# octavian-ganea/equidock_public

Measured on AMD Instinct MI355X. Metric: protein-pairs/sec (fwd+bwd) per IEGMN stack, higher is better.
Workload: dtype f32; 1 GPU; B: DB5.5-sized batch of 8 pairs x (200,200) residues, k=10, 8-layer IEGMN hdim 64, 50 heads, fp32; pairs_per_gpu=8, nodes_per_gpu=3200, edges_per_gpu=32000, layers=8, parallelism=dp1, weights=PyTorch default init (seed 0), ROT key/query x40 (SURVEY.md section 8c), svd_guard_pairs=0, launch_mode=hipGraph replay

## Files before the change

equidock_public_amd/_lib.py:

```python
import ctypes as C
import os

import torch

HERE = os.path.dirname(os.path.abspath(__file__))
LIB_PATH = os.path.join(HERE, 'libequidock_hip.so')
if os.environ.get('EQD_EXP_LIBRARY'):
    LIB_PATH = os.environ['EQD_EXP_LIBRARY']

EQD_MAX_SRC = 6
ABI_VERSION = 9
PARAMS_PER_LAYER = 19
GLOBAL_PARAMS = 5

c_float_p = C.POINTER(C.c_float)
c_int_p = C.POINTER(C.c_int32)


class EqdGraph(C.Structure):
    _fields_ = [('n_pairs', C.c_int32), ('n_lig', C.c_int32), ('n_rec', C.c_int32), ('n_nodes', C.c_int32),
                ('n_edges', C.c_int32), ('n_tiles', C.c_int32), ('n_att_items', C.c_int32), ('max_seg', C.c_int32),
                ('seg_off', C.c_void_p), ('src', C.c_void_p), ('dst', C.c_void_p), ('rowptr', C.c_void_p),
                ('csc_ptr', C.c_void_p), ('csc_eid', C.c_void_p), ('tile_node', C.c_void_p),
                ('att_items', C.c_void_p), ('res_id', C.c_void_p), ('mu_r_norm', C.c_void_p), ('he', C.c_void_p),
# ... 61 lines not shown
                ('dbc1', C.c_void_p), ('dwc2', C.c_void_p), ('dbc2', C.c_void_p)]


_lib = None
_is_sim = False
profiling = False


class EquidockHipError(RuntimeError):
    pass


def _declare(lib):
    lib.eqd_abi_version.restype = C.c_int
    lib.eqd_last_error.restype = C.c_char_p
    lib.eqd_tile_edges.restype = C.c_int
    lib.eqd_is_simulator.restype = C.c_int
    lib.eqd_model_saved_bytes.restype = C.c_size_t
    lib.eqd_model_scratch_bytes.restype = C.c_size_t
    lib.eqd_atb_partial_bytes.restype = C.c_size_t
    lib.eqd_edge_message_bwd_workspace_bytes.restype = C.c_size_t
    lib.eqd_keypoint_pool_bwd_workspace_bytes.restype = C.c_size_t
    lib.eqd_clash_workspace_bytes.restype = C.c_size_t
    lib.eqd_node_update_bwd_workspace_bytes.restype = C.c_size_t
    lib.eqd_cross_attention_bwd_ds_workspace_bytes.restype = C.c_size_t
    lib.eqd_profile_name.restype = C.c_char_p
    lib.eqd_profile_us.restype = C.c_float
    lib.eqd_tunables_reload.restype = None
    for name in ('eqd_model_layer_state', 'eqd_model_lrelu_signs', 'eqd_model_head_backward', 'eqd_profile_begin', 'eqd_profile_end', 'eqd_profile_mark', 'eqd_ctx_create', 'eqd_ctx_destroy', 'eqd_model_check', 'eqd_model_forward', 'eqd_model_backward', 'eqd_linear', 'eqd_atb',
                 'eqd_edge_message_fwd', 'eqd_edge_message_bwd', 'eqd_edge_message_bwd_kernel_only',
                 'eqd_cross_attention_fwd', 'eqd_cross_attention_fwd_bf16', 'eqd_cross_attention_bwd_bf16',
                 'eqd_cross_attention_bwd', 'eqd_cross_attention_bwd_ds',
           'eqd_keypoint_pool_fwd', 'eqd_keypoint_pool_bwd', 'eqd_kabsch_fwd', 'eqd_kabsch_bwd',
                 'eqd_rigid_apply_fwd', 'eqd_rigid_apply_bwd', 'eqd_pair_losses_fwd', 'eqd_pair_losses_bwd', 'eqd_scalar_loss', 'eqd_pocket_ot_cost',
                 'eqd_pocket_ot_fwd', 'eqd_pocket_ot_bwd', 'eqd_rigid_augment', 'eqd_protein_graph_distances',
                 'eqd_protein_graph_select', 'eqd_protein_graph_edges', 'eqd_clash_iterations', 'eqd_dropout_pack_edges', 'eqd_dropout_draw',
                 'eqd_node_update_fwd', 'eqd_node_update_bwd', 'eqd_selftest_lane_exchanges'):
        getattr(lib, name).restype = C.c_int


EXPORTS = ('eqd_model_layer_state', 'eqd_model_lrelu_signs', 'eqd_model_head_backward', 'eqd_profile_begin', 'eqd_profile_end', 'eqd_profile_mark', 'eqd_profile_name', 'eqd_profile_us', 'eqd_ctx_create', 'eqd_ctx_destroy', 'eqd_abi_version', 'eqd_last_error', 'eqd_tile_edges', 'eqd_is_simulator', 'eqd_model_saved_bytes', 'eqd_model_saved_layout',
           'eqd_model_scratch_bytes', 'eqd_model_check', 'eqd_model_forward', 'eqd_model_backward', 'eqd_linear',
           'eqd_atb_partial_bytes', 'eqd_atb', 'eqd_edge_message_fwd', 'eqd_edge_message_bwd_workspace_bytes',
           'eqd_edge_message_bwd', 'eqd_edge_message_bwd_kernel_only', 'eqd_cross_attention_fwd',
           'eqd_cross_attention_bwd', 'eqd_cross_attention_bwd_ds', 'eqd_cross_attention_bwd_ds_workspace_bytes', 'eqd_cross_attention_fwd_bf16', 'eqd_cross_attention_bwd_bf16',
           'eqd_keypoint_pool_fwd', 'eqd_keypoint_pool_bwd',
           'eqd_keypoint_pool_bwd_workspace_bytes',
           'eqd_kabsch_fwd', 'eqd_kabsch_bwd', 'eqd_rigid_apply_fwd', 'eqd_rigid_apply_bwd', 'eqd_pair_losses_fwd',
           'eqd_pair_losses_bwd', 'eqd_scalar_loss', 'eqd_pocket_ot_cost', 'eqd_pocket_ot_fwd', 'eqd_pocket_ot_bwd',
           'eqd_rigid_augment', 'eqd_protein_graph_distances', 'eqd_protein_graph_select', 'eqd_protein_graph_edges',
           'eqd_clash_workspace_bytes', 'eqd_clash_iterations', 'eqd_dropout_pack_edges', 'eqd_dropout_draw',
           'eqd_tunables_reload', 'eqd_node_update_fwd', 'eqd_node_update_bwd_workspace_bytes', 'eqd_node_update_bwd',
           'eqd_selftest_lane_exchanges', 'eqd_chain_resident_proj_launches', 'eqd_selftest_node_chain_fwd', 'eqd_model_node_state',
           'eqd_chain_resident_wide_launches')


def load_library():
    global _lib, _is_sim
    if _lib is not None:
        return _lib
    if not os.path.exists(LIB_PATH):
        raise EquidockHipError(
            f"{LIB_PATH} is missing: build it with `python -m equidock_public_amd.build` (hipcc, gfx950). "
            "There is no CPU fallback for the IEGMN hot path.")
    lib = C.CDLL(LIB_PATH)
    _declare(lib)
    if lib.eqd_abi_version() != ABI_VERSION:
        raise EquidockHipError(f"ABI version mismatch: library {lib.eqd_abi_version()} != {ABI_VERSION}")
    _lib, _is_sim = lib, bool(lib.eqd_is_simulator())
    return _lib


def load_library_for_testing(path):
    global _lib, _is_sim
    lib = C.CDLL(path)
    _declare(lib)
    _lib, _is_sim = lib, bool(lib.eqd_is_simulator())
    return _lib


def unload_for_testing():
    global _lib, _is_sim
    _lib, _is_sim = None, False


tunables_generation = 0


def reload_tunables():
    global tunables_generation
    tunables_generation += 1
    if _lib is not None:
        _lib.eqd_tunables_reload()


def is_simulator():
    return _is_sim


def check(rc):
    if rc != 0:
        raise EquidockHipError(f"libequidock_hip error {rc}: {_lib.eqd_last_error().decode()}")


def require_device(t, what='tensor'):
    if _is_sim:
        if t.is_cuda:
# ... 62 lines not shown
```

equidock_public_amd/csrc/eqd_driver.hip:

```cpp
#include "eqd_common.h"

#include <vector>

#include <string.h>

namespace {

enum {
    P_W1 = 0, P_B1, P_LNG, P_LNB, P_W2, P_B2, P_WQ, P_WK, P_WV, P_WN1, P_BN1, P_NLG, P_NLB, P_WN2, P_BN2,
    P_WC1, P_BC1, P_WC2, P_BC2
};
enum { G_EMB = 0, G_WK, G_WQ, G_WM, G_BM };

struct Dims {
    int N, E, B, K, L, d0, dh;
    int d_in(int l) const { return l == 0 ? d0 : dh; }
    int d_att(int l) const { return (d_in(l) + 15) / 16 * 16; }
    int ldw1(int l) const { return 2 * d_in(l) + 27 + 15; }
    int ldwn(int l) const { return d0 + 2 * d_in(l) + dh; }
};

Dims make_dims(const EqdModelDesc* m, const EqdGraph* g) {
    Dims D;
    D.N = g->n_nodes; D.E = g->n_edges; D.B = g->n_pairs; D.K = m->n_heads; D.L = m->n_layers;
// ... 1178 lines not shown
    nc.dHout = d_h_out; nc.Wn2 = p->Wn2; nc.Wn1 = p->Wn1; nc.y_act = y_act; nc.ln_g = p->ln_g; nc.drop_mul = p->drop_mul;
    nc.dz = W.dz; nc.lnp = W.ln_part; nc.d_aggr_msg = d_aggr_msg; nc.d_aggr_cross = aggr_cross ? d_aggr_cross : nullptr;
    nc.dh0acc = d_h0; nc.d_h = d_h;
    EqdChainJob cj[EQD_CHAIN_MAXJOBS];
    const int nj = node_bwd_chain(nc, cj);
    int nb = 0;
    RC(eqd_launch_rowchain(cj, nj, rows, st, &nb));
    EqdRedSeg segs[2] = {{W.ln_part, nb, 256, d, grads->dln_g, 0, 0, 0}, {W.ln_part + 128, nb, 256, d, grads->dln_b, 0, 0, 0}};
    RC(eqd_launch_reduce_segments(segs, 2, st));
    EqdAtbJob jobs[8];
    int na = 0;
    node_update_atb_jobs(rows, p, h, aggr_msg, aggr_cross, h0, a1n, d_h_out, W.dz, grads, jobs, &na);
    return eqd_atb(jobs, na, W.atb_part, W.atb_bytes, st);
}

extern "C" int eqd_selftest_node_chain_bwd(const EqdNodeChainBwdTest* t, int* partial_rows, void* stream) {
    if (!t || !partial_rows || !t->dH_above || !t->Wn2 || !t->Wn1 || !t->y_act || !t->ln_g || !t->dz || !t->ln_part ||
        !t->d_aggr_msg || !t->d_aggr_cross || !t->dh0acc || (t->with_dh && !t->dH)) {
        eqd_set_error("eqd_selftest_node_chain_bwd: NULL argument");
        return EQD_ERR_NULL;
    }
    if (t->rows <= 0 || t->d0 < 64 || t->d0 > 80) {
        eqd_set_error("eqd_selftest_node_chain_bwd: rows=%d d0=%d", t->rows, t->d0);
        return EQD_ERR_SHAPE;
    }
    g_bf16_mode = 0;
    const int d = 64;
    EqdLinJob dhj;
    if (t->with_dh) {
        dhj = lin_job(t->rows, d, t->dH, d, t->slope, t->ln_eps);
        for (int s = 0; s < 6; ++s) {
            if (!t->dh_X[s] || !t->dh_W[s]) {
                eqd_set_error("eqd_selftest_node_chain_bwd: NULL dh source %d", s);
                return EQD_ERR_NULL;
            }
            lin_src(dhj, s, t->dh_X[s], d, d, t->dh_W[s], 1, t->dh_wcs[s]);
        }
        dhj.nsrc = 6;
        dhj.R = t->dH_above; dhj.ldr = d; dhj.beta = 1.f - t->skip_weight_h;
    }
    NodeBwdChain nc;
    nc.N = t->rows; nc.d = d; nc.da = d; nc.d0 = t->d0; nc.d_emb = 64; nc.ldn = t->d0 + 2 * d + 64; nc.dh_width = d;
    nc.slope = t->slope; nc.eps = t->ln_eps; nc.alpha = t->skip_weight_h;
    nc.dh = t->with_dh ? &dhj : nullptr;
    nc.dHout = t->with_dh ? t->dH : t->dH_above;
    nc.Wn2 = t->Wn2; nc.Wn1 = t->Wn1; nc.y_act = t->y_act; nc.ln_g = t->ln_g; nc.drop_mul = t->drop_mul;
    nc.dz = t->dz; nc.lnp = t->ln_part; nc.d_aggr_msg = t->d_aggr_msg; nc.d_aggr_cross = t->d_aggr_cross; nc.dh0acc = t->dh0acc;
    nc.d_h = nullptr;
    EqdChainJob cj[8];
    const int nj = node_bwd_chain(nc, cj);
    return eqd_launch_rowchain(cj, nj, t->rows, (hipStream_t)stream, partial_rows);
}

extern "C" int eqd_selftest_node_chain_fwd(const EqdNodeChainFwdTest* t, void* stream) {
    if (!t || !t->h || !t->aggr_msg || !t->aggr_cross || !t->h0 || !t->Wn1 || !t->Bn1 || !t->ln_g || !t->ln_b || !t->Wn2 ||
        !t->Bn2 || !t->a1n || !t->y_act || !t->h_out) {
        eqd_set_error("eqd_selftest_node_chain_fwd: NULL argument");
        return EQD_ERR_NULL;
    }
    if (t->rows <= 0 || t->d0 < 64 || t->d0 > 80 || (t->form != 0 && t->form != 1 && t->form != 5)) {
        eqd_set_error("eqd_selftest_node_chain_fwd: rows=%d d0=%d form=%d", t->rows, t->d0, t->form);
        return EQD_ERR_SHAPE;
    }
    if (t->form == 5 ? (!t->W1 || !t->B1 || !t->WQ || !t->WK || !t->WV || !t->P || !t->Q || !t->qa || !t->ka || !t->va)
                     : (t->form == 1 && (!t->WM || !t->BM || !t->hm))) {
        eqd_set_error("eqd_selftest_node_chain_fwd: NULL argument of a carried job");
        return EQD_ERR_NULL;
    }
    g_bf16_mode = 0;
    const int d = 64;
    NodeFwdChain fc;
    fc.N = t->rows; fc.d = d; fc.da = d; fc.d0 = t->d0; fc.dh = d; fc.ldn = t->d0 + 2 * d + 64; fc.ld_a1n = d;
    fc.slope = t->slope; fc.eps = t->ln_eps; fc.skip = t->skip_weight_h;
    fc.h = t->h; fc.aggr_msg = t->aggr_msg; fc.aggr_cross = t->aggr_cross; fc.h0 = t->h0;
    fc.Wn1 = t->Wn1; fc.Bn1 = t->Bn1; fc.ln_g = t->ln_g; fc.ln_b = t->ln_b; fc.Wn2 = t->Wn2; fc.Bn2 = t->Bn2;
    fc.drop_mul = t->drop_mul;
    fc.a1n = t->a1n; fc.y_act = t->y_act; fc.h_out = t->h_out; fc.a1n_b = nullptr; fc.hb_out = nullptr;
    fc.next = nullptr; fc.head = nullptr;
    NodePre np;
    EqdLinJob jm;
    if (t->form == 5) {
        np.N = t->rows; np.d = d; np.da = d; np.ldw1 = 2 * d; np.slope = t->slope; np.eps = t->ln_eps; np.cross = true;
        np.W1 = t->W1; np.B1 = t->B1; np.WQ = t->WQ; np.WK = t->WK; np.WV = t->WV;
        np.P = t->P; np.Q = t->Q; np.qa = t->qa; np.ka = t->ka; np.va = t->va;
        np.qa_b = np.ka_b = np.va_b = nullptr;
        fc.next = &np;
    } else if (t->form == 1) {
        jm = lin_job(t->rows, 64, t->hm, 64, t->slope, t->ln_eps);
        lin_src(jm, 0, t->h_out, d, d, t->WM, d, 1);
        jm.nsrc = 1; jm.bias = t->BM; jm.act = 1;
        jm.mul = t->head_mul; jm.ld_mul = 64;
        fc.head = &jm;
    }
    EqdChainJob cj[EQD_CHAIN_MAXJOBS];
    const int nj = node_fwd_chain(fc, cj);
    return eqd_launch_rowchain(cj, nj, t->rows, (hipStream_t)stream);
}
```

equidock_public_amd/csrc/eqd_node_kernels.hip:

```cpp
#include "eqd_common.h"
#include "eqd_linear_inl.h"
#include "eqd_rowwave_inl.h"
#include "eqd_rowres_inl.h"
#include "eqd_rowres80_inl.h"
#include "eqd_chainres_inl.h"
#include "eqd_chainres_wide_inl.h"
#include "eqd_gather_inl.h"

#include <atomic>
#include <mutex>
#include <vector>

#include <stdarg.h>
#include <stdio.h>
#include <stdlib.h>
#include <string.h>

static thread_local char g_err[512] = "";

void eqd_set_error(const char* fmt, ...) {
    va_list ap;
    va_start(ap, fmt);
    vsnprintf(g_err, sizeof(g_err), fmt, ap);
    va_end(ap);
// ... 499 lines not shown
    *(f32x4*)&Lb[0][out_l][l15 * LIN_S + f0] = z;
    if (rv && jY) *(EQD_GAS f4v*)&jY[(size_t)rowi * ldy + f0] = z;
    float v8[8];
#pragma unroll
    for (int r = 0; r < 4; ++r) {
        v8[r] = o[r] * xh[r];
        v8[4 + r] = o[r];
    }
    const bool b3 = (l15 & 8) != 0, b2 = (l15 & 4) != 0, b1 = (l15 & 2) != 0;
    float w4[4], w2[2];
#pragma unroll
    for (int i = 0; i < 4; ++i) w4[i] = (b3 ? v8[i + 4] : v8[i]) + lane_xor<8>(b3 ? v8[i] : v8[i + 4]);
#pragma unroll
    for (int i = 0; i < 2; ++i) w2[i] = (b2 ? w4[i + 2] : w4[i]) + lane_xor<4>(b2 ? w4[i] : w4[i + 2]);
    float w1 = (b1 ? w2[1] : w2[0]) + lane_xor<2>(b1 ? w2[0] : w2[1]);
    w1 += lane_xor<1>(w1);
    if ((l15 & 1) == 0) {
        const int idx = l15 >> 1;
        jaux[(size_t)blockIdx.x * 256 + (idx < 4 ? 0 : 128) + f0 + (idx & 3)] = w1;
    }
}
struct LnBwd64Desc {
    const JobW& W;
    bool have_y;
    f32x4 yp;
#define LJ(f) JW_OFF(EqdLinJob, f)
    __device__ __forceinline__ int rows() const { return jw_i(W, LJ(rows)); }
    __device__ __forceinline__ int src_l() const { return jw_i(W, JW_OFF(EqdChainJob, src_local)); }
    __device__ __forceinline__ int out_l() const { return jw_i(W, JW_OFF(EqdChainJob, out_local)); }
    __device__ __forceinline__ float slope() const { return jw_f(W, LJ(slope)); }
    __device__ __forceinline__ float ln_eps() const { return jw_f(W, LJ(ln_eps)); }
    __device__ __forceinline__ f32x4 gam(int f0) const { return *(const EQD_GAS f4v*)(jw_p<const float>(W, LJ(ln_g)) + f0); }
    __device__ __forceinline__ f32x4 y_act(int row, int f0) const {
        if (have_y) return yp;
        const int ldx = jw_i(W, LJ(s) + JW_OFF(EqdLinSrc, ldx));
        return *(const EQD_GAS f4v*)(jw_p<const float>(W, LJ(s) + JW_OFF(EqdLinSrc, X)) + (size_t)row * ldx + f0);
    }
    __device__ __forceinline__ float* Y() const { return jw_p<float>(W, LJ(Y)); }
    __device__ __forceinline__ int ldy() const { return jw_i(W, LJ(ldy)); }
    __device__ __forceinline__ float* aux() const { return jw_p<float>(W, JW_OFF(EqdChainJob, aux)); }
    __device__ __forceinline__ f32x4 mul(int row, int f0) const {
        f32x4 mulv = {1.f, 1.f, 1.f, 1.f};
        if (const float* const jmul = jw_p<const float>(W, LJ(mul)))
            mulv = *(const EQD_GAS f4v*)(jmul + (size_t)row * jw_i(W, LJ(ld_mul)) + f0);
        return mulv;
    }
#undef LJ
};
__device__ __forceinline__ void chain_lnbwd64(const JobW& W, float (*Lb)[LIN_LOCALS][16 * LIN_S], float (*stat)[EQD_WAVES][16],
                                              int row0, bool have_y, f32x4 yp) {
    chain_lnbwd64_t(LnBwd64Desc{W, have_y, yp}, Lb, stat, row0);
}
#include "eqd_chainres_bwd_inl.h"

template <int RT>
__device__ __forceinline__ void chain_lnbwd(const EqdChainJob& C, float (*Lb)[LIN_LOCALS][16 * LIN_S], float (*red)[256],
                                            int row0) {
    const EqdLinJob& J = C.lin;
    const EQD_GAS float* const jlng = (const EQD_GAS float*)uni(J.ln_g);
    const EQD_GAS float* const jX = (const EQD_GAS float*)uni(J.s[0].X);
    EQD_GAS float* const jY = (EQD_GAS float*)uni(J.Y);
    EQD_GAS float* const jaux = (EQD_GAS float*)uni(C.aux);
    const EQD_GAS float* const jmul = (const EQD_GAS float*)uni(J.mul);
    const int ld_mul = uni(J.ld_mul);
    const int rows = uni(J.rows), ldx = uni(J.s[0].ldx), ldy = uni(J.ldy), src_l = uni(C.src_local[0]), out_l = uni(C.out_local);
    const float slope = uni(J.slope), ln_eps = uni(J.ln_eps);
    const int t = threadIdx.x, lane = t & 63, wave = t >> 6;
    const int d = uni(J.M);
    const int f0 = lane, f1 = lane + 64;
    const bool v0 = f0 < d, v1 = f1 < d;
    const float g0 = v0 ? jlng[f0] : 0.f, g1 = v1 ? jlng[f1] : 0.f;
    const float invd = 1.f / (float)d;
    float dg0 = 0.f, dg1 = 0.f, db0 = 0.f, db1 = 0.f;
    float y0s[RT][4], y1s[RT][4];
#pragma unroll
    for (int rt = 0; rt < RT; ++rt)
#pragma unroll
        for (int rr = 0; rr < 4; ++rr) {
            int row = row0 + 16 * rt + 4 * wave + rr;
            row = row < rows ? row : rows - 1;
            const size_t o = (size_t)row * ldx;
            y0s[rt][rr] = jX[o + (v0 ? f0 : 0)];
            y1s[rt][rr] = jX[o + (v1 ? f1 : 0)];
        }
#pragma unroll
    for (int rt = 0; rt < RT; ++rt) {
        const float* __restrict__ din = Lb[rt][src_l];
        float* __restrict__ dout = Lb[rt][out_l];
#pragma unroll
        for (int rr = 0; rr < 4; ++rr) {
            const int lr = 4 * wave + rr;
            const int row = row0 + 16 * rt + lr;
            const bool rv = row < rows;
            const float y0 = (rv && v0) ? y0s[rt][rr] : 0.f, y1 = (rv && v1) ? y1s[rt][rr] : 0.f;
            const float o0 = (rv && v0) ? din[lr * LIN_S + f0] : 0.f, o1 = (rv && v1) ? din[lr * LIN_S + f1] : 0.f;
            const float mean = wave_sum(y0 + y1) * invd;
            const float c0 = v0 ? y0 - mean : 0.f, c1 = v1 ? y1 - mean : 0.f;
            const float rstd = 1.f / sqrtf(wave_sum(c0 * c0 + c1 * c1) * invd + ln_eps);
            const float xh0 = c0 * rstd, xh1 = c1 * rstd;
            const float dx0 = o0 * g0, dx1 = o1 * g1;
            const float s1 = wave_sum(dx0 + dx1) * invd;
            const float s2 = wave_sum(dx0 * xh0 + dx1 * xh1) * invd;
            float z0 = rstd * (dx0 - s1 - xh0 * s2) * lrelu_grad(y0, slope);
            float z1 = rstd * (dx1 - s1 - xh1 * s2) * lrelu_grad(y1, slope);
            if (jmul) {
                const size_t mo = (size_t)(rv ? row : rows - 1) * ld_mul;
// ... 314 lines not shown
            return false;
        for (int s = 0; s < nsrc; ++s)
            if (!J.s[s].W || J.s[s].mask || J.s[s].K != 64 || J.s[s].w_rs != 1) return false;
        return true;
    };
    auto src = [](const EqdLinSrc& S) { return CrbSrc{S.X, S.W, S.ldx, S.w_cs}; };
    auto out = [](const EqdLinJob& J) { return CrbOut{J.Y, J.R, J.ldy, J.ldr, J.alpha, J.beta}; };
    memset(&A, 0, sizeof(A));
    A.rows = rows;
    int at = 0;
    if (dh) {
        const EqdChainJob& C = jobs[at++];
        if (!plain(C, 6) || C.out_local != 2 || !C.lin.Y || !C.lin.R) return false;
        for (int s = 0; s < 6; ++s) {
            if (!C.lin.s[s].X || C.src_local[s] >= 0) return false;
            A.dh[s] = src(C.lin.s[s]);
        }
        A.dho = out(C.lin);
    }
    {
        const EqdChainJob& C = jobs[at++];
        if (!plain(C, 1) || C.out_local != 0 || C.lin.Y || C.lin.R) return false;
        if (dh ? C.src_local[0] != 2 : (C.src_local[0] >= 0 || !C.lin.s[0].X)) return false;
        A.a = src(C.lin.s[0]);
        A.a_alpha = C.lin.alpha;
        A.a_beta = C.lin.beta;
    }
    {
        const EqdChainJob& C = jobs[at++];
        const EqdLinJob& J = C.lin;
        if (C.type != 1 || J.bf16 || J.rows != rows || J.M != 64 || C.src_local[0] != 0 || C.out_local != 1 || !J.s[0].X ||
            !J.ln_g || !J.Y || !C.aux)
            return false;
        A.y_act = J.s[0].X; A.ld_y = J.s[0].ldx;
        A.ln_g = J.ln_g;
        A.mul = J.mul; A.ld_mul = J.ld_mul;
        A.dz = J.Y; A.ld_dz = J.ldy;
        A.aux = C.aux;
        A.slope = J.slope; A.ln_eps = J.ln_eps;
    }
    for (int j = 0; j < 3; ++j) {
        const EqdChainJob& C = jobs[at++];
        if (!plain(C, 1) || C.src_local[0] != 1 || C.out_local >= 0 || !C.lin.Y) return false;
        if (C.lin.R && !(dh && j == 2 && C.lin.R == C.lin.Y && C.lin.ldr == C.lin.ldy)) return false;
        A.x[j] = src(C.lin.s[0]);
        A.xo[j] = out(C.lin);
        if (j > 0 && (A.x[j].W != A.x[j - 1].W + 64 || A.x[j].wcs != A.x[j - 1].wcs)) return false;
    }
    return true;
}
static std::atomic<long long> g_chain_resident_bwd_launches{0};
extern "C" long long eqd_chain_resident_bwd_launches(void) { return g_chain_resident_bwd_launches.load(); }

enum RowBody {
    ROW_NONE,
    ROW_RES80,
    ROW_RES, ROW_WAVE,
    ROW_CRF0, ROW_CRF1, ROW_CRF5,
    ROW_CRW,
    ROW_CRB, ROW_CRB_DH,
    ROW_CHAIN
};
struct RowPlan {
    RowBody body;
    int grid;
    int tps;
    bool bf;
    int rt, occ;
    union {
        ChainResFwdArg f;
        ChainResWideArg w;
        ChainResBwdArg b;
    } res;
    std::atomic<long long>* count[2];
};
static RowPlan row_plan(const EqdChainJob* jobs, int njobs, int rows, bool chain, bool wide_ok) {
    RowPlan P;
    memset(&P, 0, sizeof(P));
    P.bf = njobs > 0 && jobs[0].lin.bf16;
    const bool rw = rw_eligible(jobs, njobs, rows);
    if (!rw && rw80_eligible(jobs, njobs, rows)) P.body = ROW_RES80;
    else if (rw) P.body = rw_mode(rows) == 2 && rr_single_tile(jobs, njobs) ? ROW_RES : ROW_WAVE;
    if (P.body == ROW_WAVE) P.grid = rw_blocks(rows);
    else if (P.body != ROW_NONE) { P.tps = rr_tiles_per_wg(rows); P.grid = rr_blocks(rows); }
    if (P.body != ROW_NONE || !chain) return P;
    P.grid = eqd_rowchain_blocks(rows);
    const int occ = rowchain_occ_forced();
    if (cr_rows_ok(rows, occ)) {
        int np = 0;
        if (crf_pack(jobs, njobs, rows, P.res.f, np)) {
            P.body = np == 5 ? ROW_CRF5 : np == 1 ? ROW_CRF1 : ROW_CRF0;
            P.count[0] = &g_chain_resident_launches;
            if (np) P.count[1] = &g_chain_resident_proj_launches;
            return P;
        }
        if (wide_ok && crw_pack(jobs, njobs, rows, P.res.w)) {
            P.body = ROW_CRW; P.count[0] = &g_chain_resident_wide_launches;
            return P;
        }
        if (crb_pack(jobs, njobs, rows, P.res.b)) {
            P.body = njobs == 6 ? ROW_CRB_DH : ROW_CRB; P.count[0] = &g_chain_resident_bwd_launches;
            return P;
        }
    }
    P.body = ROW_CHAIN;
    P.rt = eqd_row_tiles(rows);
    P.occ = P.rt == 2 ? 1 : occ > 0 ? occ : (P.grid <= eqd_num_cus() ? 1 : 2);
    return P;
}
template <class... A>
static void row_go(void (*kernel)(A...), const RowPlan& P, int threads, hipStream_t st, A... args) {
    hipLaunchKernelGGL(kernel, dim3(P.grid), dim3(threads), 0, st, args...);
}
static int row_launch(const RowPlan& P, const EqdChainArg& arg, hipStream_t st) {
    const char* family = "k_rowchain";
    switch (P.body) {
    case ROW_NONE: return EQD_ERR_UNSUPPORTED;
    case ROW_RES80: row_go(k_rowres80, P, 64 * RR_WAVES, st, arg, P.tps); family = "k_rowres"; break;
    case ROW_RES:
        if (P.bf) row_go(k_rowres<true>, P, 64 * RR_WAVES, st, arg, P.tps);
        else row_go(k_rowres<false>, P, 64 * RR_WAVES, st, arg, P.tps);
        family = "k_rowres";
        break;
    case ROW_WAVE:
        if (P.bf) row_go(k_rowwave<true>, P, 64 * RW_WAVES, st, arg);
        else row_go(k_rowwave<false>, P, 64 * RW_WAVES, st, arg);
        family = "k_rowwave";
        break;
    case ROW_CRF0: row_go(k_rowchain_res_fwd<0>, P, EQD_BLOCK, st, P.res.f); break;
    case ROW_CRF1: row_go(k_rowchain_res_fwd<1>, P, EQD_BLOCK, st, P.res.f); break;
    case ROW_CRF5: row_go(k_rowchain_res_fwd<5>, P, EQD_BLOCK, st, P.res.f); break;
    case ROW_CRW: row_go(k_rowchain_res_fwd_wide, P, EQD_BLOCK, st, P.res.w); break;
    case ROW_CRB: row_go(k_rowchain_res_bwd<false>, P, EQD_BLOCK, st, P.res.b); break;
    case ROW_CRB_DH: row_go(k_rowchain_res_bwd<true>, P, EQD_BLOCK, st, P.res.b); break;
    case ROW_CHAIN:
        if (P.rt == 2 && P.bf) row_go(k_rowchain<2, true, 1>, P, EQD_BLOCK, st, arg);
        else if (P.rt == 2) row_go(k_rowchain<2, false, 1>, P, EQD_BLOCK, st, arg);
        else if (P.bf && P.occ == 1) row_go(k_rowchain<1, true, 1>, P, EQD_BLOCK, st, arg);
        else if (P.bf) row_go(k_rowchain<1, true, 2>, P, EQD_BLOCK, st, arg);
        else if (P.occ == 1) row_go(k_rowchain<1, false, 1>, P, EQD_BLOCK, st, arg);
        else row_go(k_rowchain<1, false, 2>, P, EQD_BLOCK, st, arg);
        break;
    }
    for (int i = 0; i < 2; ++i)
        if (P.count[i]) P.count[i]->fetch_add(1);
    return eqd_check_launch(family);
}

int eqd_launch_rowchain(const EqdChainJob* jobs, int njobs, int rows, hipStream_t st, int* partial_rows, bool wide_ok) {
    if (njobs <= 0 || njobs > EQD_CHAIN_MAXJOBS) {
        eqd_set_error("eqd_launch_rowchain: %d jobs (1..%d)", njobs, EQD_CHAIN_MAXJOBS);
        return EQD_ERR_SHAPE;
    }
    if (rows <= 0) return EQD_OK;
    EqdChainArg arg;
    memset(&arg, 0, sizeof(arg));
    for (int i = 0; i < njobs; ++i) {
        arg.j[i] = jobs[i];
        const EqdLinJob& J = jobs[i].lin;
        if (J.M < 4 || J.M > 80 || J.rows != rows) {
            eqd_set_error("eqd_launch_rowchain: job %d has M=%d rows=%d (chain rows %d)", i, J.M, J.rows, rows);
            return EQD_ERR_SHAPE;
        }
        if (jobs[i].type == 0)
            if (int e = lin_check_sources(J)) return e;
        for (int s = 0; s < J.nsrc; ++s)
            if (jobs[i].src_local[s] >= 0 && (J.s[s].K > 80 || jobs[i].src_local[s] >= LIN_LOCALS)) {
                eqd_set_error("eqd_launch_rowchain: LDS-resident source wider than %d or tile index >= %d", 80, LIN_LOCALS);
                return EQD_ERR_SHAPE;
            }
    }
    arg.njobs = njobs;
    chain_links(arg);
    for (int i = 0; i < njobs; ++i)
        if (jobs[i].out_local >= LIN_LOCALS) {
            eqd_set_error("eqd_launch_rowchain: LDS tile index %d >= %d", jobs[i].out_local, LIN_LOCALS);
            return EQD_ERR_SHAPE;
        }
    const RowPlan P = row_plan(jobs, njobs, rows, true, wide_ok);
    if (partial_rows) *partial_rows = P.grid;
    return row_launch(P, arg, st);
}

extern "C" int eqd_linear(const EqdLinJob* jobs, int njobs, void* stream) {
    if (!jobs || njobs <= 0) {
        eqd_set_error("eqd_linear: no jobs");
        return EQD_ERR_NULL;
// ... 1016 lines not shown
```

include/equidock_hip.h:

```cpp
#ifndef EQUIDOCK_HIP_H
#define EQUIDOCK_HIP_H

#include <stddef.h>
#include <stdint.h>

#ifdef __cplusplus
extern "C" {
#endif

#define EQD_ABI_VERSION 9
#define EQD_TILE_EDGES 32
#define EQD_ATT_BLOCK 32
#define EQD_MAX_SRC 6
#define EQD_PARAMS_PER_LAYER 19
#define EQD_GLOBAL_PARAMS 5

enum {
    EQD_OK = 0,
    EQD_ERR_NULL = 1,
    EQD_ERR_SHAPE = 2,
    EQD_ERR_UNSUPPORTED = 3,
    EQD_ERR_WORKSPACE = 4,
    EQD_ERR_LAUNCH = 5
};

int eqd_abi_version(void);
const char* eqd_last_error(void);
int eqd_tile_edges(void);
int eqd_is_simulator(void);
void eqd_tunables_reload(void);
long long eqd_chain_resident_launches(void);
long long eqd_chain_resident_bwd_launches(void);
typedef struct EqdNodeChainBwdTest {
    int32_t rows, with_dh, d0;
    float skip_weight_h, slope, ln_eps;
    const float* dh_X[6];
    const float* dh_W[6];
    int32_t dh_wcs[6];
    const float* dH_above;
    float* dH;
    const float* Wn2;
    const float* Wn1;
    const float* y_act;
    const float* ln_g;
    const float* drop_mul;
    float* dz;
    float* ln_part;
    float* d_aggr_msg;
    float* d_aggr_cross;
    float* dh0acc;
} EqdNodeChainBwdTest;
int eqd_selftest_node_chain_bwd(const EqdNodeChainBwdTest* t, int* partial_rows , void* stream);
long long eqd_chain_resident_proj_launches(void);
long long eqd_chain_resident_wide_launches(void);
typedef struct EqdNodeChainFwdTest {
    int32_t rows, d0, form;
    float skip_weight_h, slope, ln_eps;
    const float* h; const float* aggr_msg; const float* aggr_cross; const float* h0;
    const float* Wn1; const float* Bn1; const float* ln_g; const float* ln_b; const float* Wn2; const float* Bn2;
    const float* drop_mul;
    float* a1n; float* y_act; float* h_out;
    const float* W1; const float* B1; const float* WQ; const float* WK; const float* WV;
    float* P; float* Q; float* qa; float* ka; float* va;
    const float* WM; const float* BM; const float* head_mul ; float* hm;
} EqdNodeChainFwdTest;
int eqd_selftest_node_chain_fwd(const EqdNodeChainFwdTest* t, void* stream);
int eqd_selftest_lane_exchanges(const float* in256, int* mismatch, float* out256, void* stream);

int eqd_profile_begin(void* stream, int max_launches);
int eqd_profile_end(void);
int eqd_profile_mark(const char* label);
const char* eqd_profile_name(int i);
float eqd_profile_us(int i);

typedef struct EqdGraph {
    int32_t n_pairs, n_lig, n_rec, n_nodes, n_edges, n_tiles, n_att_items, max_seg;
    const int32_t* seg_off;
    const int32_t* src;
    const int32_t* dst;
    const int32_t* rowptr;
    const int32_t* csc_ptr;
    const int32_t* csc_eid;
    const int32_t* tile_node;
    const int32_t* att_items;
    const int32_t* res_id;
    const float* mu_r_norm;
    const float* he;
    const float* x0;
    const uint16_t* he_bf16;
} EqdGraph;

typedef struct EqdModelDesc {
    int32_t n_layers;
    int32_t d_emb;
    int32_t d_hid;
    int32_t use_mean_node_features;
    int32_t edge_feats;
    int32_t n_heads;
    int32_t cross_msgs, use_dist_in_layers, use_edge_features;
    float skip_weight_h, x_connection_init, lrelu_slope, ln_eps;
    int32_t svd_seed;
    int32_t storage_bf16;
} EqdModelDesc;

typedef struct EqdDropout {
    float p;
    const uint32_t* edge_z1;
// ... 219 lines not shown
```

Before: 8357 pairs/s.

## Add resident wide backward node-chain kernel for layer-0 width-69 chain

Adds a specialised fused kernel that runs the six-job node-update backward chain for the layer with 69-wide input (layer 0) in one launch. It keeps weights and row tiles in LDS and handles the extra 5 columns beyond 64 with separate MFMA paths. The previous path was the generic k_rowchain. The fused kernel targets the generic kernel's launch overhead and its intermediate global traffic, at the cost of heavy LDS use (occupancy 1) and a narrow pattern match. Activation depends on the EQD_CHAIN_RESIDENT_WIDE_BWD switch and on the chain matching exactly.

```diff
diff --git a/equidock_public_amd/_lib.py b/equidock_public_amd/_lib.py
--- a/equidock_public_amd/_lib.py
+++ b/equidock_public_amd/_lib.py
@@ -137,7 +137,7 @@
            'eqd_clash_workspace_bytes', 'eqd_clash_iterations', 'eqd_dropout_pack_edges', 'eqd_dropout_draw',
            'eqd_tunables_reload', 'eqd_node_update_fwd', 'eqd_node_update_bwd_workspace_bytes', 'eqd_node_update_bwd',
            'eqd_selftest_lane_exchanges', 'eqd_chain_resident_proj_launches', 'eqd_selftest_node_chain_fwd', 'eqd_model_node_state',
-           'eqd_chain_resident_wide_launches')
+           'eqd_chain_resident_wide_launches', 'eqd_chain_resident_wide_bwd_launches', 'eqd_selftest_node_chain_bwd_wide')
 
 
 def load_library():
diff --git a/equidock_public_amd/csrc/eqd_chainres_bwd_wide_inl.h b/equidock_public_amd/csrc/eqd_chainres_bwd_wide_inl.h
--- /dev/null
+++ b/equidock_public_amd/csrc/eqd_chainres_bwd_wide_inl.h
@@ -0,0 +1,272 @@
+#pragma once
+#include "eqd_chainres_bwd_inl.h"
+
+struct ChainResBwdWideArg {
+    ChainResBwdArg c;
+    int M, pad_to;
+};
+struct alignas(1024) ChainResBwdWideSmem {
+    float W[6][EQD_WAVES][CRB_SLAB];
+    float X[7][CR_XTILE];
+    float B4[2][512];
+    float Kr[1024];
+};
+
+__device__ __forceinline__ float crbw_b4(const float* __restrict__ img, int k, int l15) {
+    const float v = img[8 * k + (l15 < 4 ? l15 : 7)];
+    return l15 < 5 ? v : 0.f;
+}
+__device__ __forceinline__ void crbw_mma(f32x4 (&acc)[2], f32x4 (&acc2)[2], const float* __restrict__ slab,
+                                         const float* __restrict__ b4, const f32x4 (&b)[4], bool own1, int lane, int l15, int g) {
+    f32x4 a[4], a4[4];
+#pragma unroll
+    for (int q = 0; q < 4; ++q)
+#pragma unroll
+        for (int j = 0; j < 4; ++j) a[q][j] = slab[256 * q + 64 * j + lane];
+    if (own1) {
+#pragma unroll
+        for (int q = 0; q < 4; ++q)
+#pragma unroll
+            for (int j = 0; j < 4; ++j) a4[q][j] = crbw_b4(b4, 16 * q + 4 * g + j, l15);
+    }
+#ifndef EQD_HOSTSIM
+    __builtin_amdgcn_sched_barrier(0);
+#endif
+#pragma unroll
+    for (int q = 0; q < 4; ++q) {
+        acc[0] = mfma4(a[q][0], b[q][0], acc[0]);
+        acc2[0] = mfma4(a[q][1], b[q][1], acc2[0]);
+        acc[0] = mfma4(a[q][2], b[q][2], acc[0]);
+        acc2[0] = mfma4(a[q][3], b[q][3], acc2[0]);
+    }
+    if (own1) {
+#pragma unroll
+        for (int q = 0; q < 4; ++q) {
+            acc[1] = mfma4(a4[q][0], b[q][0], acc[1]);
+            acc2[1] = mfma4(a4[q][1], b[q][1], acc2[1]);
+            acc[1] = mfma4(a4[q][2], b[q][2], acc[1]);
+            acc2[1] = mfma4(a4[q][3], b[q][3], acc2[1]);
+        }
+    }
+}
+__device__ __forceinline__ void crbw_mma_rem(f32x4 (&acc)[2], f32x4 (&acc2)[2], const float* __restrict__ kr,
+                                             const float* __restrict__ kr4, const f32x4 b, bool own1, int wave, int l15, int g) {
+    f32x4 a, a4 = f4zero();
+#pragma unroll
+    for (int j = 0; j < 4; ++j) {
+        const int k = 4 * g + j, kc = k < 5 ? k : 4;
+        const float v = kr[64 * kc + 16 * wave + l15];
+        a[j] = k < 5 ? v : 0.f;
+    }
+    acc[0] = mfma4(a[0], b[0], acc[0]);
+    acc2[0] = mfma4(a[1], b[1], acc2[0]);
+    acc[0] = mfma4(a[2], b[2], acc[0]);
+    acc2[0] = mfma4(a[3], b[3], acc2[0]);
+    if (own1) {
+#pragma unroll
+        for (int j = 0; j < 4; ++j) {
+            const int k = 4 * g + j, kc = k < 5 ? k : 4;
+            const float v = crbw_b4(kr4, kc, l15);
+            a4[j] = k < 5 ? v : 0.f;
+        }
+        acc[1] = mfma4(a4[0], b[0], acc[1]);
+        acc2[1] = mfma4(a4[1], b[1], acc2[1]);
+        acc[1] = mfma4(a4[2], b[2], acc[1]);
+        acc2[1] = mfma4(a4[3], b[3], acc2[1]);
+    }
+}
+
+__device__ __forceinline__ void crbw_lnbwd(const ChainResBwdArg& A, const int d, float (*Lb)[LIN_LOCALS][16 * LIN_S],
+                                           float (*red)[256], int row0, float g0r, float g1r, const float (&y0s)[4],
+                                           const float (&y1s)[4], const float (&m0s)[4], const float (&m1s)[4]) {
+    EQD_GAS float* const jY = (EQD_GAS float*)A.dz;
+    EQD_GAS float* const jaux = (EQD_GAS float*)A.aux;
+    const int rows = A.rows, ldy = A.ld_dz;
+    const float slope = A.slope, ln_eps = A.ln_eps;
+    const int t = threadIdx.x, lane = t & 63, wave = t >> 6;
+    const int f0 = lane, f1 = lane + 64;
+    const bool v0 = f0 < d, v1 = f1 < d;
+    const float g0 = v0 ? g0r : 0.f, g1 = v1 ? g1r : 0.f;
+    const float invd = 1.f / (float)d;
+    float dg0 = 0.f, dg1 = 0.f, db0 = 0.f, db1 = 0.f;
+    const float* __restrict__ din = Lb[0][0];
+    float* __restrict__ dout = Lb[0][1];
+#pragma unroll
+    for (int rr = 0; rr < 4; ++rr) {
+        const int lr = 4 * wave + rr;
+        const int row = row0 + lr;
+        const bool rv = row < rows;
+        const float y0 = (rv && v0) ? y0s[rr] : 0.f, y1 = (rv && v1) ? y1s[rr] : 0.f;
+        const float o0 = (rv && v0) ? din[lr * LIN_S + f0] : 0.f, o1 = (rv && v1) ? din[lr * LIN_S + f1] : 0.f;
+        const float mean = wave_sum(y0 + y1) * invd;
+        const float c0 = v0 ? y0 - mean : 0.f, c1 = v1 ? y1 - mean : 0.f;
+        const float rstd = 1.f / sqrtf(wave_sum(c0 * c0 + c1 * c1) * invd + ln_eps);
+        const float xh0 = c0 * rstd, xh1 = c1 * rstd;
+        const float dx0 = o0 * g0, dx1 = o1 * g1;
+        const float s1 = wave_sum(dx0 + dx1) * invd;
+        const float s2 = wave_sum(dx0 * xh0 + dx1 * xh1) * invd;
+        float z0 = rstd * (dx0 - s1 - xh0 * s2) * lrelu_grad(y0, slope);
+        float z1 = rstd * (dx1 - s1 - xh1 * s2) * lrelu_grad(y1, slope);
+        if (A.mul) {
+            z0 *= m0s[rr];
+            z1 *= m1s[rr];
+        }
+        if (v0) dout[lr * LIN_S + f0] = rv ? z0 : 0.f;
+        if (v1) dout[lr * LIN_S + f1] = rv ? z1 : 0.f;
+        if (rv && jY) {
+            if (v0) jY[(size_t)row * ldy + f0] = z0;
+            if (v1) jY[(size_t)row * ldy + f1] = z1;
+        }
+        if (rv) {
+            dg0 += o0 * xh0;
+            dg1 += o1 * xh1;
+            db0 += o0;
+            db1 += o1;
+        }
+    }
+    red[wave][lane] = dg0;
+    red[wave][64 + lane] = dg1;
+    red[wave][128 + lane] = db0;
+    red[wave][192 + lane] = db1;
+    __syncthreads();
+    jaux[(size_t)blockIdx.x * 256 + t] = red[0][t] + red[1][t] + red[2][t] + red[3][t];
+}
+
+__global__ __launch_bounds__(EQD_BLOCK, 1) void k_rowchain_res_bwd_wide(ChainResBwdWideArg AW) {
+    __shared__ ChainResBwdWideSmem S;
+    __shared__ __attribute__((aligned(16))) float Lb[1][LIN_LOCALS][16 * LIN_S];
+    __shared__ float red[EQD_WAVES][256];
+    const ChainResBwdArg& A = AW.c;
+    const int t = threadIdx.x, lane = t & 63, wave = t >> 6, l15 = lane & 15, g = lane >> 4;
+    const int row0 = (int)blockIdx.x * 16, rows = A.rows, M = AW.M;
+    for (int i = t; i < LIN_LOCALS * 16 * LIN_S; i += EQD_BLOCK) (&Lb[0][0][0])[i] = 0.f;
+    const int f0 = 16 * wave + 4 * g;
+    const int rowi = row0 + l15;
+    const bool rv = rowi < rows;
+    const int rowe = rv ? rowi : rows - 1;
+    const int fb = lane + 64 < M ? lane + 64 : 0;
+    float g0r = ((const EQD_GAS float*)A.ln_g)[lane], g1r = ((const EQD_GAS float*)A.ln_g)[fb];
+    float y0s[4], y1s[4], m0s[4], m1s[4];
+    {
+        const EQD_GAS float* const mp = (const EQD_GAS float*)(A.mul ? A.mul : A.ln_g);
+        const int ldm = A.mul ? A.ld_mul : 0;
+#pragma unroll
+        for (int rr = 0; rr < 4; ++rr) {
+            int row = row0 + 4 * wave + rr;
+            row = row < rows ? row : rows - 1;
+            const size_t o = (size_t)row * A.ld_y, mo = (size_t)row * ldm;
+            y0s[rr] = ((const EQD_GAS float*)A.y_act)[o + lane];
+            y1s[rr] = ((const EQD_GAS float*)A.y_act)[o + fb];
+            m0s[rr] = mp[mo + lane];
+            m1s[rr] = mp[mo + fb];
+        }
+    }
+    f32x4 res2 = *(const EQD_GAS f4v*)(A.xo[2].R + (size_t)rowe * A.xo[2].ldr + f0);
+    f32x4 acc = f4zero(), acc2 = f4zero();
+#pragma unroll
+    for (int s = 0; s < 6; ++s) crb_copy_rows(A.dh[s].X, A.dh[s].ldx, S.X[s], row0, rows, wave, lane);
+    crb_copy_rows(A.dho.R, A.dho.ldr, S.X[6], row0, rows, wave, lane);
+#pragma unroll
+    for (int c = 0; c < 6; ++c) crb_copy_chunk(A.dh[c].W, A.dh[c].wcs, S.W[c][wave], wave, lane);
+    {
+        const bool n2 = wave < 2;
+        const float* const Wb = n2 ? A.a.W : A.x[1].W;
+        const int wcs = n2 ? A.a.wcs : A.x[1].wcs;
+        const int k = 32 * (wave & 1) + (lane >> 1);
+        glds16(Wb + (size_t)k * wcs + ((lane & 1) ? M - 4 : 64), &S.B4[wave >> 1][256 * (wave & 1)]);
+    }
+    {
+        int G = 64 * wave + lane;
+        G = G < 249 ? G : 249;
+        const bool blk = G < 240;
+        const int j = blk ? G / 80 : 1;
+        const int r = blk ? (G % 80) >> 4 : (G - 240) >> 1;
+        const int m = blk ? 4 * (G & 15) : ((G & 1) ? M - 4 : 64);
+        const int c0 = j == 0 ? 0 : (j == 1 ? 64 : 64 + M);
+        glds16(A.x[0].W + (size_t)(64 + r) * A.x[0].wcs + c0 + m, &S.Kr[256 * wave]);
+    }
+    vm_wait<26>();
+    lds_barrier();
+    vm_wait<22>();
+    crb_mma<false>(acc, acc2, S.W[0][wave], S.X[0], lane, l15, g);
+    lds_reads_done();
+    crb_copy_chunk(A.a.W, A.a.wcs, S.W[0][wave], wave, lane);
+    vm_wait<22>();
+    crb_mma<false>(acc, acc2, S.W[1][wave], S.X[1], lane, l15, g);
+    lds_reads_done();
+    crb_copy_chunk(A.x[0].W, A.x[0].wcs, S.W[1][wave], wave, lane);
+    vm_wait<22>();
+    crb_mma<false>(acc, acc2, S.W[2][wave], S.X[2], lane, l15, g);
+    lds_reads_done();
+    crb_copy_chunk(A.x[1].W, A.x[1].wcs, S.W[2][wave], wave, lane);
+    vm_wait<22>();
+    crb_mma<false>(acc, acc2, S.W[3][wave], S.X[3], lane, l15, g);
+    lds_reads_done();
+    crb_copy_chunk(A.x[2].W, A.x[2].wcs, S.W[3][wave], wave, lane);
+    vm_wait<22>();
+    crb_mma<false>(acc, acc2, S.W[4][wave], S.X[4], lane, l15, g);
+    vm_wait<18>();
+    crb_mma<false>(acc, acc2, S.W[5][wave], S.X[5], lane, l15, g);
+    {
+        const f32x4 resd = *(const f32x4*)&S.X[6][cr_at(l15, 4 * wave + g)];
+        const f32x4 yv = crb_epilogue(acc, acc2, A.dho.alpha, A.dho.beta, resd);
+        if (rv) *(EQD_GAS f4v*)&A.dho.Y[(size_t)rowi * A.dho.ldy + f0] = yv;
+        *(f32x4*)&Lb[0][2][l15 * LIN_S + f0] = yv;
+    }
+    vm_wait<0>();
+    keep_after_wait(g0r); keep_after_wait(g1r); keep_after_wait(res2);
+#pragma unroll
+    for (int rr = 0; rr < 4; ++rr) {
+        keep_after_wait(y0s[rr]); keep_after_wait(y1s[rr]); keep_after_wait(m0s[rr]); keep_after_wait(m1s[rr]);
+    }
+    __syncthreads();
+    const bool own1 = wave == 0;
+    const int nf4 = M - 64 - 4 * g;
+    f32x4 av[2], av2[2], b[4];
+    av[0] = av[1] = av2[0] = av2[1] = f4zero();
+#pragma unroll
+    for (int q = 0; q < 4; ++q) b[q] = *(const f32x4*)&Lb[0][2][l15 * LIN_S + 16 * q + 4 * g];
+    crbw_mma(av, av2, S.W[0][wave], S.B4[0], b, own1, lane, l15, g);
+    *(f32x4*)&Lb[0][0][l15 * LIN_S + f0] = crb_epilogue(av[0], av2[0], A.a_alpha, A.a_beta, f4zero());
+    if (own1) {
+        const f32x4 y4 = crb_epilogue(av[1], av2[1], A.a_alpha, A.a_beta, f4zero());
+#pragma unroll
+        for (int r = 0; r < 4; ++r)
+            if (r < nf4) Lb[0][0][l15 * LIN_S + 64 + 4 * g + r] = y4[r];
+    }
+    __syncthreads();
+    crbw_lnbwd(A, M, Lb, red, row0, g0r, g1r, y0s, y1s, m0s, m1s);
+    __syncthreads();
+#pragma unroll
+    for (int q = 0; q < 4; ++q) b[q] = *(const f32x4*)&Lb[0][1][l15 * LIN_S + 16 * q + 4 * g];
+    const f32x4 brem = *(const f32x4*)&Lb[0][1][l15 * LIN_S + 64 + 4 * g];
+    {
+        av[0] = av[1] = av2[0] = av2[1] = f4zero();
+        crbw_mma(av, av2, S.W[1][wave], S.B4[1], b, false, lane, l15, g);
+        crbw_mma_rem(av, av2, &S.Kr[0], &S.Kr[960], brem, false, wave, l15, g);
+        const f32x4 yv = crb_epilogue(av[0], av2[0], A.xo[0].alpha, A.xo[0].beta, f4zero());
+        if (rv) *(EQD_GAS f4v*)&A.xo[0].Y[(size_t)rowi * A.xo[0].ldy + f0] = yv;
+    }
+    {
+        av[0] = av[1] = av2[0] = av2[1] = f4zero();
+        crbw_mma(av, av2, S.W[2][wave], S.B4[1], b, own1, lane, l15, g);
+        crbw_mma_rem(av, av2, &S.Kr[320], &S.Kr[960], brem, own1, wave, l15, g);
+        const f32x4 yv = crb_epilogue(av[0], av2[0], A.xo[1].alpha, A.xo[1].beta, f4zero());
+        if (rv) *(EQD_GAS f4v*)&A.xo[1].Y[(size_t)rowi * A.xo[1].ldy + f0] = yv;
+        if (own1) {
+            const f32x4 y4 = crb_epilogue(av[1], av2[1], A.xo[1].alpha, A.xo[1].beta, f4zero());
+#pragma unroll
+            for (int r = 0; r < 4; ++r) {
+                const int f = 64 + 4 * g + r;
+                if (rv && (r < nf4 || f < AW.pad_to)) ((EQD_GAS float*)A.xo[1].Y)[(size_t)rowi * A.xo[1].ldy + f] = r < nf4 ? y4[r] : 0.f;
+            }
+        }
+    }
+    {
+        av[0] = av[1] = av2[0] = av2[1] = f4zero();
+        crbw_mma(av, av2, S.W[3][wave], S.B4[1], b, false, lane, l15, g);
+        crbw_mma_rem(av, av2, &S.Kr[640], &S.Kr[960], brem, false, wave, l15, g);
+        const f32x4 yv = crb_epilogue(av[0], av2[0], A.xo[2].alpha, A.xo[2].beta, res2);
+        if (rv) *(EQD_GAS f4v*)&A.xo[2].Y[(size_t)rowi * A.xo[2].ldy + f0] = yv;
+    }
+}
diff --git a/equidock_public_amd/csrc/eqd_driver.hip b/equidock_public_amd/csrc/eqd_driver.hip
--- a/equidock_public_amd/csrc/eqd_driver.hip
+++ b/equidock_public_amd/csrc/eqd_driver.hip
@@ -1254,6 +1254,41 @@
     return eqd_launch_rowchain(cj, nj, t->rows, (hipStream_t)stream, partial_rows);
 }
 
+extern "C" int eqd_selftest_node_chain_bwd_wide(const EqdNodeChainBwdWideTest* t, int* partial_rows, void* stream) {
+    if (!t || !partial_rows || !t->dH_above || !t->dH || !t->Wn2 || !t->Wn1 || !t->y_act || !t->ln_g || !t->dz || !t->ln_part ||
+        !t->d_aggr_msg || !t->d_aggr_cross || !t->dh0acc) {
+        eqd_set_error("eqd_selftest_node_chain_bwd_wide: NULL argument");
+        return EQD_ERR_NULL;
+    }
+    if (t->rows <= 0) {
+        eqd_set_error("eqd_selftest_node_chain_bwd_wide: rows=%d", t->rows);
+        return EQD_ERR_SHAPE;
+    }
+    g_bf16_mode = 0;
+    const int d = 69, dh = 64;
+    EqdLinJob dhj = lin_job(t->rows, dh, t->dH, dh, t->slope, t->ln_eps);
+    for (int s = 0; s < 6; ++s) {
+        if (!t->dh_X[s] || !t->dh_W[s]) {
+            eqd_set_error("eqd_selftest_node_chain_bwd_wide: NULL dh source %d", s);
+            return EQD_ERR_NULL;
+        }
+        lin_src(dhj, s, t->dh_X[s], dh, dh, t->dh_W[s], 1, t->dh_wcs[s]);
+    }
+    dhj.nsrc = 6;
+    dhj.R = t->dH_above; dhj.ldr = dh; dhj.beta = 1.f - t->skip_weight_h;
+    NodeBwdChain nc;
+    nc.N = t->rows; nc.d = d; nc.da = 80; nc.d0 = d; nc.d_emb = 64; nc.ldn = 3 * d + 64; nc.dh_width = dh;
+    nc.slope = t->slope; nc.eps = t->ln_eps; nc.alpha = 1.f;
+    nc.dh = &dhj;
+    nc.dHout = t->dH;
+    nc.Wn2 = t->Wn2; nc.Wn1 = t->Wn1; nc.y_act = t->y_act; nc.ln_g = t->ln_g; nc.drop_mul = t->drop_mul;
+    nc.dz = t->dz; nc.lnp = t->ln_part; nc.d_aggr_msg = t->d_aggr_msg; nc.d_aggr_cross = t->d_aggr_cross; nc.dh0acc = t->dh0acc;
+    nc.d_h = nullptr;
+    EqdChainJob cj[8];
+    const int nj = node_bwd_chain(nc, cj);
+    return eqd_launch_rowchain(cj, nj, t->rows, (hipStream_t)stream, partial_rows);
+}
+
 extern "C" int eqd_selftest_node_chain_fwd(const EqdNodeChainFwdTest* t, void* stream) {
     if (!t || !t->h || !t->aggr_msg || !t->aggr_cross || !t->h0 || !t->Wn1 || !t->Bn1 || !t->ln_g || !t->ln_b || !t->Wn2 ||
         !t->Bn2 || !t->a1n || !t->y_act || !t->h_out) {
diff --git a/equidock_public_amd/csrc/eqd_node_kernels.hip b/equidock_public_amd/csrc/eqd_node_kernels.hip
--- a/equidock_public_amd/csrc/eqd_node_kernels.hip
+++ b/equidock_public_amd/csrc/eqd_node_kernels.hip
@@ -575,6 +575,7 @@
     chain_lnbwd64_t(LnBwd64Desc{W, have_y, yp}, Lb, stat, row0);
 }
 #include "eqd_chainres_bwd_inl.h"
+#include "eqd_chainres_bwd_wide_inl.h"
 
 template <int RT>
 __device__ __forceinline__ void chain_lnbwd(const EqdChainJob& C, float (*Lb)[LIN_LOCALS][16 * LIN_S], float (*red)[256],
@@ -995,6 +996,67 @@
 static std::atomic<long long> g_chain_resident_bwd_launches{0};
 extern "C" long long eqd_chain_resident_bwd_launches(void) { return g_chain_resident_bwd_launches.load(); }
 
+static bool crbw_pack(const EqdChainJob* jobs, int njobs, int rows, ChainResBwdWideArg& AW) {
+    if (njobs != 6 || !chain_resident_on() || !eqd_switch_on("EQD_CHAIN_RESIDENT_WIDE_BWD") || rw_mode(rows) != 0) return false;
+    auto plain = [&](const EqdChainJob& C, int M, int nsrc, int K, int pad_to) {
+        const EqdLinJob& J = C.lin;
+        if (C.type != 0 || J.bf16 || J.rows != rows || J.M != M || J.nsrc != nsrc || J.act || J.bias || J.ln_g || J.ln_b ||
+            J.pre_ln || J.mul || J.pad_to != pad_to || J.Yb)
+            return false;
+        for (int s = 0; s < nsrc; ++s)
+            if (!J.s[s].W || J.s[s].mask || J.s[s].K != K || J.s[s].w_rs != 1 || J.s[s].w_cs < M) return false;
+        return true;
+    };
+    auto src = [](const EqdLinSrc& S) { return CrbSrc{S.X, S.W, S.ldx, S.w_cs}; };
+    auto out = [](const EqdLinJob& J) { return CrbOut{J.Y, J.R, J.ldy, J.ldr, J.alpha, J.beta}; };
+    memset(&AW, 0, sizeof(AW));
+    ChainResBwdArg& A = AW.c;
+    A.rows = rows; AW.M = 69; AW.pad_to = 80;
+    {
+        const EqdChainJob& C = jobs[0];
+        if (!plain(C, 64, 6, 64, 0) || C.out_local != 2 || !C.lin.Y || !C.lin.R || C.lin.ldy < 64 || C.lin.ldr < 64) return false;
+        for (int s = 0; s < 6; ++s) {
+            if (!C.lin.s[s].X || C.src_local[s] >= 0 || C.lin.s[s].ldx < 64) return false;
+            A.dh[s] = src(C.lin.s[s]);
+        }
+        A.dho = out(C.lin);
+    }
+    {
+        const EqdChainJob& C = jobs[1];
+        if (!plain(C, 69, 1, 64, 0) || C.src_local[0] != 2 || C.out_local != 0 || C.lin.Y || C.lin.R) return false;
+        A.a = src(C.lin.s[0]);
+        A.a_alpha = C.lin.alpha;
+        A.a_beta = C.lin.beta;
+    }
+    {
+        const EqdChainJob& C = jobs[2];
+        const EqdLinJob& J = C.lin;
+        if (C.type != 1 || J.bf16 || J.rows != rows || J.M != 69 || C.src_local[0] != 0 || C.out_local != 1 || !J.s[0].X ||
+            J.s[0].ldx < 69 || !J.ln_g || !J.Y || J.ldy < 69 || !C.aux || (J.mul && J.ld_mul < 69))
+            return false;
+        A.y_act = J.s[0].X; A.ld_y = J.s[0].ldx;
+        A.ln_g = J.ln_g;
+        A.mul = J.mul; A.ld_mul = J.ld_mul;
+        A.dz = J.Y; A.ld_dz = J.ldy;
+        A.aux = C.aux;
+        A.slope = J.slope; A.ln_eps = J.ln_eps;
+    }
+    const int Ms[3] = {64, 69, 64}, pads[3] = {0, 80, 0};
+    for (int j = 0; j < 3; ++j) {
+        const EqdChainJob& C = jobs[3 + j];
+        if (!plain(C, Ms[j], 1, 69, pads[j]) || C.src_local[0] != 1 || C.out_local >= 0 || !C.lin.Y ||
+            C.lin.ldy < (pads[j] ? pads[j] : Ms[j]))
+            return false;
+        if (j == 2 ? !(C.lin.R && C.lin.R == C.lin.Y && C.lin.ldr == C.lin.ldy && C.lin.ldy == 69) : C.lin.R != nullptr) return false;
+        A.x[j] = src(C.lin.s[0]);
+        A.xo[j] = out(C.lin);
+        if (j > 0 && (A.x[j].W != A.x[j - 1].W + Ms[j - 1] || A.x[j].wcs != A.x[j - 1].wcs)) return false;
+    }
+    return true;
+}
+static std::atomic<long long> g_chain_resident_wide_bwd_launches{0};
+extern "C" long long eqd_chain_resident_wide_bwd_launches(void) { return g_chain_resident_wide_bwd_launches.load(); }
+
 enum RowBody {
     ROW_NONE,
     ROW_RES80,
@@ -1002,6 +1064,7 @@
     ROW_CRF0, ROW_CRF1, ROW_CRF5,
     ROW_CRW,
     ROW_CRB, ROW_CRB_DH,
+    ROW_CRBW,
     ROW_CHAIN
 };
 struct RowPlan {
@@ -1014,6 +1077,7 @@
         ChainResFwdArg f;
         ChainResWideArg w;
         ChainResBwdArg b;
+        ChainResBwdWideArg bw;
     } res;
     std::atomic<long long>* count[2];
 };
@@ -1045,6 +1109,10 @@
             P.body = njobs == 6 ? ROW_CRB_DH : ROW_CRB; P.count[0] = &g_chain_resident_bwd_launches;
             return P;
         }
+        if (crbw_pack(jobs, njobs, rows, P.res.bw)) {
+            P.body = ROW_CRBW; P.count[0] = &g_chain_resident_wide_bwd_launches;
+            return P;
+        }
     }
     P.body = ROW_CHAIN;
     P.rt = eqd_row_tiles(rows);
@@ -1076,6 +1144,7 @@
     case ROW_CRW: row_go(k_rowchain_res_fwd_wide, P, EQD_BLOCK, st, P.res.w); break;
     case ROW_CRB: row_go(k_rowchain_res_bwd<false>, P, EQD_BLOCK, st, P.res.b); break;
     case ROW_CRB_DH: row_go(k_rowchain_res_bwd<true>, P, EQD_BLOCK, st, P.res.b); break;
+    case ROW_CRBW: row_go(k_rowchain_res_bwd_wide, P, EQD_BLOCK, st, P.res.bw); break;
     case ROW_CHAIN:
         if (P.rt == 2 && P.bf) row_go(k_rowchain<2, true, 1>, P, EQD_BLOCK, st, arg);
         else if (P.rt == 2) row_go(k_rowchain<2, false, 1>, P, EQD_BLOCK, st, arg);
diff --git a/include/equidock_hip.h b/include/equidock_hip.h
--- a/include/equidock_hip.h
+++ b/include/equidock_hip.h
@@ -53,6 +53,27 @@
 int eqd_selftest_node_chain_bwd(const EqdNodeChainBwdTest* t, int* partial_rows , void* stream);
 long long eqd_chain_resident_proj_launches(void);
 long long eqd_chain_resident_wide_launches(void);
+long long eqd_chain_resident_wide_bwd_launches(void);
+typedef struct EqdNodeChainBwdWideTest {
+    int32_t rows;
+    float skip_weight_h, slope, ln_eps;
+    const float* dh_X[6];
+    const float* dh_W[6];
+    int32_t dh_wcs[6];
+    const float* dH_above;
+    float* dH;
+    const float* Wn2;
+    const float* Wn1;
+    const float* y_act;
+    const float* ln_g;
+    const float* drop_mul;
+    float* dz;
+    float* ln_part;
+    float* d_aggr_msg;
+    float* d_aggr_cross;
+    float* dh0acc;
+} EqdNodeChainBwdWideTest;
+int eqd_selftest_node_chain_bwd_wide(const EqdNodeChainBwdWideTest* t, int* partial_rows , void* stream);
 typedef struct EqdNodeChainFwdTest {
     int32_t rows, d0, form;
     float skip_weight_h, slope, ln_eps;
```

After: 8529 pairs/s, median of 6. 1.02x the previous value.
